# dke-lab/dgll

Hardware: AMD Instinct MI355X
Metric: aggregated edges/sec + epoch time, 3-layer GraphSAGE ogbn-products, 1/2/4/8 GPU (higher is better)
Workload: dtype bf16

## Files before the change

dgll_amd/csrc/gather.hpp:

```cpp
#pragma once
#include "common.hpp"

int dgll_spmm_csr_impl(void* stream, const dgll_csr_plan* plan, const int64_t* rowptr, const int32_t* col,
                       const float* val, const void* X, int64_t ldx, int x_dtype, void* Y, int64_t ldy,
                       int y_dtype, int64_t n_rows, int64_t n_cols, int feat, int reduce, int epilogue,
                       const float* bias, void* workspace, size_t workspace_bytes, const float* row_scale, int accumulate,
                       const void* gate, int64_t ldg, int only_long);

namespace dgll {

template <typename XT, int EPV, int LPR, bool HAS_VAL, int U>
__device__ __forceinline__ void gather_edges(const int32_t* __restrict__ col, const float* __restrict__ val,
                                             const XT* __restrict__ xcol, int64_t ldx, int64_t b, int64_t e,
                                             int lane, float (&acc)[EPV], bool preloaded = false, int first_col = 0,
                                             float first_val = 0.0f) {
    typedef VecIO<XT, EPV> IO;
    constexpr int SLOTS = kWave / LPR;
    const int slot = lane / LPR;

    int my_col = first_col;
    float my_val = first_val;
    if (!preloaded) {
        my_col = 0;
        my_val = 0.0f;
        if (b + lane < e) {
            my_col = __builtin_nontemporal_load(col + b + lane);
            if (HAS_VAL) my_val = __builtin_nontemporal_load(val + b + lane);
        }
    }
    for (int64_t k0 = b; k0 < e; k0 += kWave) {
        const int64_t left = e - k0;
        const int nb = left < kWave ? (int)left : kWave;
        const int cur_col = my_col;
        const float cur_val = my_val;
        const int64_t kn = k0 + kWave + lane;
        if (kn < e) {
            my_col = __builtin_nontemporal_load(col + kn);
            if (HAS_VAL) my_val = __builtin_nontemporal_load(val + kn);
        }
        const uint32_t ld32 = (uint32_t)ldx;
        int j = 0;
        for (; j + SLOTS * U <= nb; j += SLOTS * U) {
            int c[U];
            float w[U];
#pragma unroll
            for (int u = 0; u < U; ++u) {
                const int src = j + u * SLOTS + slot;
                c[u] = __shfl(cur_col, src);
                w[u] = HAS_VAL ? __shfl(cur_val, src) : 1.0f;
            }
            typename IO::raw_t v[U];
#pragma unroll
            for (int u = 0; u < U; ++u) v[u] = IO::load(xcol + (uint64_t)(uint32_t)c[u] * ld32);
#pragma unroll
            for (int u = 0; u < U; ++u) {
                float f[EPV];
                IO::unpack(v[u], f);
#pragma unroll
                for (int i = 0; i < EPV; ++i) acc[i] = HAS_VAL ? fmaf(w[u], f[i], acc[i]) : acc[i] + f[i];
            }
        }
        if (j < nb) {
            int c[U];
            float w[U];
            bool ok[U];
#pragma unroll
            for (int u = 0; u < U; ++u) {
                const int idx = j + u * SLOTS + slot;
                ok[u] = idx < nb;
                const int src = ok[u] ? idx : nb - 1;
                c[u] = __shfl(cur_col, src);
                w[u] = HAS_VAL ? __shfl(cur_val, src) : 1.0f;
            }
            typename IO::raw_t v[U];
#pragma unroll
            for (int u = 0; u < U; ++u) v[u] = IO::load(xcol + (uint64_t)(uint32_t)c[u] * ld32);
#pragma unroll
            for (int u = 0; u < U; ++u) {
                float f[EPV];
                IO::unpack(ok[u] ? v[u] : IO::zero(), f);
#pragma unroll
                for (int i = 0; i < EPV; ++i) acc[i] = HAS_VAL ? fmaf(w[u], f[i], acc[i]) : acc[i] + f[i];
            }
        }
    }
#pragma unroll
    for (int off = LPR; off < kWave; off <<= 1) {
#pragma unroll
        for (int i = 0; i < EPV; ++i) acc[i] += __shfl_xor(acc[i], off);
    }
}

}
```

dgll_amd/csrc/spmm.hip:

```cpp
#include <algorithm>
#include <vector>

#include "common.hpp"
#include "gather.hpp"
#include <type_traits>

namespace dgll {

struct LongRow { int64_t row, begin, end; };

__global__ void find_long_rows_kernel(const int64_t* __restrict__ rowptr, int64_t n_rows, int threshold,
                                      LongRow* __restrict__ out, unsigned long long* __restrict__ count,
                                      unsigned long long capacity) {
    for (int64_t r = blockIdx.x * (int64_t)blockDim.x + threadIdx.x; r < n_rows; r += (int64_t)gridDim.x * blockDim.x) {
        const int64_t b = rowptr[r], e = rowptr[r + 1];
        if (e - b > threshold) {
            const unsigned long long at = atomicAdd(count, 1ull);
            if (at < capacity) out[at] = LongRow{r, b, e};
        }
    }
}

constexpr int64_t kFlatRowCost = 4;
__global__ void flat_row0_kernel(const int64_t* __restrict__ rowptr, int64_t n_rows, int64_t cost_per_wave, int64_t n_flat,
// ... 102 lines not shown
        if (vec_bias) v += bv[i];
        else if ((epilogue & DGLL_EPI_BIAS) && c0 + i < feat) v += bias[c0 + i];
        if (epilogue & DGLL_EPI_RELU) v = fmaxf(v, 0.0f);
        acc[i] = v;
    }
    if constexpr (EXTRA) {
        if (gate) {
            float gv[EPV];
            if (full) gatev.unpack(gv);
#pragma unroll
            for (int i = 0; i < EPV; ++i) {
                if (full) { if (!(gv[i] > 0.0f)) acc[i] = 0.0f; }
                else if (c0 + i < feat && !(load_one<YT>(gate + c0 + i) > 0.0f)) acc[i] = 0.0f;
            }
        }
        if (accumulate == 2) {
            float p[EPV];
            if (full) prev.unpack(p);
#pragma unroll
            for (int i = 0; i < EPV; ++i)
                if (full) acc[i] += p[i];
                else if (c0 + i < feat) acc[i] += load_one<YT>(y + c0 + i);
        }
    }
    if (full) {
        if constexpr (std::is_same<YT, bf16_t>::value && EPV == 8) {
            VecIO<YT, EPV>::store_nt(y + c0, acc);
        } else {
            VecIO<YT, EPV>::store(y + c0, acc);
        }
    } else {
#pragma unroll
        for (int i = 0; i < EPV; ++i)
            if (c0 + i < feat) store_one<YT>(y + c0 + i, acc[i]);
    }
}

template <typename XT, typename YT, int EPV, int LPR, bool HAS_VAL, int U, bool EXTRA, bool PF = false>
__global__ __launch_bounds__(kBlock) void spmm_csr_kernel(const SpmmArgs a) {
    const int lane = lane_id();
    const int wave = __builtin_amdgcn_readfirstlane((int)(threadIdx.x >> 6));
    const int sub = lane % LPR;
    const int c0 = ((int)blockIdx.y * LPR + sub) * EPV;
    const bool col_ok = c0 < a.feat;
    const XT* xcol = static_cast<const XT*>(a.X) + (col_ok ? c0 : 0);
    uint32_t bid = blockIdx.x;

    if (bid < a.chunk_blocks) {
        const int64_t chunk = __builtin_amdgcn_readfirstlane((int)(bid * kWavesPerBlock + wave));
        if (chunk >= a.n_chunks) return;
        float acc[EPV];
#pragma unroll
        for (int i = 0; i < EPV; ++i) acc[i] = 0.0f;
        gather_edges<XT, EPV, LPR, HAS_VAL, U>(a.col, a.val, xcol, a.ldx, uniform64(a.chunk_begin[chunk]),
                                               uniform64(a.chunk_end[chunk]), lane, acc);
        if (lane < LPR && col_ok) {
            float* w = a.ws + chunk * a.ws_ld + c0;
#pragma unroll
            for (int i = 0; i < EPV; ++i) w[i] = acc[i];
        }
        return;
    }

    bid -= a.chunk_blocks;
    if (a.flags & 1) bid = xcd_remap(bid, a.row_blocks);
    const int64_t row0 = ((int64_t)bid * kWavesPerBlock + wave) * a.rows_per_wave;
    constexpr bool pf = PF;
    int64_t nb_ = 0, ne_ = 0;
    int ncol = 0;
    float nval = 0.0f;
    if (pf && row0 < a.n_rows) {
        nb_ = uniform64(a.rowptr[row0]); ne_ = uniform64(a.rowptr[row0 + 1]);
        if (nb_ + lane < ne_) {
            ncol = __builtin_nontemporal_load(a.col + nb_ + lane);
            if (HAS_VAL) nval = __builtin_nontemporal_load(a.val + nb_ + lane);
        }
    }
    for (int r = 0; r < a.rows_per_wave; ++r) {
        const int64_t row = row0 + r;
        if (row >= a.n_rows) return;
        int64_t b, e;
        int fcol = 0;
        float fval = 0.0f;
        if (pf) {
            b = nb_; e = ne_; fcol = ncol; fval = nval;
            if (r + 1 < a.rows_per_wave && row + 1 < a.n_rows) {
                nb_ = e; ne_ = uniform64(a.rowptr[row + 2]);
                ncol = 0; nval = 0.0f;
                if (nb_ + lane < ne_) {
                    ncol = __builtin_nontemporal_load(a.col + nb_ + lane);
                    if (HAS_VAL) nval = __builtin_nontemporal_load(a.val + nb_ + lane);
                }
            }
        } else {
            b = uniform64(a.rowptr[row]); e = uniform64(a.rowptr[row + 1]);
        }
        if (a.threshold > 0 && e - b > a.threshold) continue;
        if constexpr (EXTRA) {
            if (a.accumulate == 2 && e == b) continue;
        }
        float acc[EPV];
#pragma unroll
        for (int i = 0; i < EPV; ++i) acc[i] = 0.0f;
        YT* yrow = static_cast<YT*>(a.Y) + row * a.ldy;
        const bool writer = lane < LPR && col_ok;
        const bool full = c0 + EPV <= a.feat;
        RowVec<YT, EPV> prev, gatev;
        const YT* grow = nullptr;
        if constexpr (EXTRA) {
            grow = a.gate ? static_cast<const YT*>(a.gate) + row * a.ldg : nullptr;
        }
        gather_edges<XT, EPV, LPR, HAS_VAL, U>(a.col, a.val, xcol, a.ldx, b, e, lane, acc, pf, fcol, fval);
        if constexpr (EXTRA) {
            if (writer && full) {
                if (a.accumulate) prev.load(yrow + c0);
                if (grow) gatev.load(grow + c0);
            }
        }
        if (writer) {
            const float scale = a.row_scale ? a.row_scale[row]
                                            : ((a.reduce == DGLL_REDUCE_MEAN && e > b) ? 1.0f / (float)(e - b) : 1.0f);
            finish_row<YT, EPV, EXTRA>(yrow, c0, a.feat, scale, a.epilogue, a.bias, acc, a.accumulate, grow, full, prev, gatev);
        }
    }
}

template <typename XT, typename YT, int EPV, int LPR, bool HAS_VAL, int U, bool EXTRA>
__global__ __launch_bounds__(kBlock) void spmm_csr_flat_kernel(const SpmmArgs a) {
    typedef VecIO<XT, EPV> IO;
    constexpr int SLOTS = kWave / LPR, G = SLOTS * U;
    const int lane = lane_id();
    const int wave = __builtin_amdgcn_readfirstlane((int)(threadIdx.x >> 6));
    const int sub = lane % LPR, slot = lane / LPR;
    const int c0 = ((int)blockIdx.y * LPR + sub) * EPV;
    const bool col_ok = c0 < a.feat;
    const XT* xcol = static_cast<const XT*>(a.X) + (col_ok ? c0 : 0);
    uint32_t bid = blockIdx.x;

    if (bid < a.chunk_blocks) {
        const int64_t chunk = __builtin_amdgcn_readfirstlane((int)(bid * kWavesPerBlock + wave));
        if (chunk >= a.n_chunks) return;
        float acc[EPV];
#pragma unroll
        for (int i = 0; i < EPV; ++i) acc[i] = 0.0f;
        gather_edges<XT, EPV, LPR, HAS_VAL, U>(a.col, a.val, xcol, a.ldx, uniform64(a.chunk_begin[chunk]),
                                               uniform64(a.chunk_end[chunk]), lane, acc);
        if (lane < LPR && col_ok) {
            float* w = a.ws + chunk * a.ws_ld + c0;
#pragma unroll
            for (int i = 0; i < EPV; ++i) w[i] = acc[i];
        }
        return;
    }
    bid -= a.chunk_blocks;
    const int64_t w = (int64_t)bid * kWavesPerBlock + wave;
    if (w >= a.n_flat) return;
    int64_t r = uniform64(a.flat_row0[w]);
    const int64_t r_end = uniform64(a.flat_row0[w + 1]);
    if (r >= r_end) return;
    int64_t rb = uniform64(a.rowptr[r]), re = uniform64(a.rowptr[r + 1]);
    const int64_t p_end = uniform64(a.rowptr[r_end]);
    int64_t p = rb;
    const bool writer = lane < LPR && col_ok;
    const bool full = c0 + EPV <= a.feat;
    const uint32_t ld32 = (uint32_t)a.ldx;
    const int thr = a.threshold;
    float acc[EPV];
#pragma unroll
    for (int i = 0; i < EPV; ++i) acc[i] = 0.0f;
    bool stop = false;

    auto flush = [&]() {
#pragma unroll
        for (int off = LPR; off < kWave; off <<= 1) {
#pragma unroll
            for (int i = 0; i < EPV; ++i) acc[i] += __shfl_xor(acc[i], off);
        }
        bool emit = writer;
        if constexpr (EXTRA) {
            if (a.accumulate == 2 && re == rb) emit = false;
        }
        if (emit) {
            YT* yrow = static_cast<YT*>(a.Y) + r * a.ldy;
            RowVec<YT, EPV> prev, gatev;
            const YT* grow = nullptr;
            if constexpr (EXTRA) {
                grow = a.gate ? static_cast<const YT*>(a.gate) + r * a.ldg : nullptr;
                if (full) {
                    if (a.accumulate) prev.load(yrow + c0);
                    if (grow) gatev.load(grow + c0);
                }
            }
            const float scale = a.row_scale ? a.row_scale[r]
                                            : ((a.reduce == DGLL_REDUCE_MEAN && re > rb) ? 1.0f / (float)(re - rb) : 1.0f);
            finish_row<YT, EPV, EXTRA>(yrow, c0, a.feat, scale, a.epilogue, a.bias, acc, a.accumulate, grow, full, prev, gatev);
        }
#pragma unroll
        for (int i = 0; i < EPV; ++i) acc[i] = 0.0f;
        ++r;
        rb = re;
        if (r < r_end) {
            re = uniform64(a.rowptr[r + 1]);
            stop = thr > 0 && re - rb > thr;
        } else {
            stop = true;
        }
    };

    stop = thr > 0 && re - rb > thr;
    int my_col = 0, nx_col = 0;
    float my_val = 0.0f, nx_val = 0.0f;
    int64_t nx_p = -1;
    while (r < r_end) {
        if (stop) {
            p = re;
            ++r;
            rb = re;
            stop = false;
            if (r < r_end) {
                re = uniform64(a.rowptr[r + 1]);
                stop = thr > 0 && re - rb > thr;
            }
            continue;
        }
        if (re == rb) {
            flush();
            continue;
        }
        const int64_t left = p_end - p;
        const int nb = left < kWave ? (int)left : kWave;
        if (nx_p == p) {
            my_col = nx_col;
            my_val = nx_val;
        } else {
            my_col = 0;
            my_val = 0.0f;
            if (lane < nb) {
                my_col = __builtin_nontemporal_load(a.col + p + lane);
                if (HAS_VAL) my_val = __builtin_nontemporal_load(a.val + p + lane);
            }
        }
        nx_p = p + kWave;
        nx_col = 0;
        nx_val = 0.0f;
        if (nx_p + lane < p_end) {
            nx_col = __builtin_nontemporal_load(a.col + nx_p + lane);
            if (HAS_VAL) nx_val = __builtin_nontemporal_load(a.val + nx_p + lane);
        }
        int j = 0;
        while (j < nb && !stop) {
            const int64_t q0 = p + j;
            const int64_t in_row = re - q0;
            int cnt = nb - j < G ? nb - j : G;
            if (in_row < cnt) cnt = (int)in_row;
            if (cnt == G) {
                int c[U];
                float wv[U];
#pragma unroll
                for (int u = 0; u < U; ++u) {
                    const int src = j + u * SLOTS + slot;
                    c[u] = __shfl(my_col, src);
                    wv[u] = HAS_VAL ? __shfl(my_val, src) : 1.0f;
                }
                typename IO::raw_t v[U];
#pragma unroll
                for (int u = 0; u < U; ++u) v[u] = IO::load(xcol + (uint64_t)(uint32_t)c[u] * ld32);
#pragma unroll
                for (int u = 0; u < U; ++u) {
                    float f[EPV];
                    IO::unpack(v[u], f);
#pragma unroll
                    for (int i = 0; i < EPV; ++i) acc[i] = HAS_VAL ? fmaf(wv[u], f[i], acc[i]) : acc[i] + f[i];
                }
            } else {
                int c[U];
                float wv[U];
                bool ok[U];
#pragma unroll
                for (int u = 0; u < U; ++u) {
                    const int idx = u * SLOTS + slot;
                    ok[u] = idx < cnt;
                    const int src = j + (ok[u] ? idx : cnt - 1);
                    c[u] = __shfl(my_col, src);
                    wv[u] = HAS_VAL ? __shfl(my_val, src) : 1.0f;
                }
                typename IO::raw_t v[U];
#pragma unroll
                for (int u = 0; u < U; ++u) v[u] = IO::load(xcol + (uint64_t)(uint32_t)c[u] * ld32);
#pragma unroll
                for (int u = 0; u < U; ++u) {
                    float f[EPV];
                    IO::unpack(ok[u] ? v[u] : IO::zero(), f);
#pragma unroll
                    for (int i = 0; i < EPV; ++i) acc[i] = HAS_VAL ? fmaf(wv[u], f[i], acc[i]) : acc[i] + f[i];
                }
            }
            j += cnt;
            if (q0 + cnt == re) {
                flush();
                while (!stop && re == rb) flush();
            }
        }
        p = stop ? rb : p + j;
    }
}

template <typename XT, typename YT, int EPV, int LPR, bool HAS_VAL, bool EXTRA>
__global__ __launch_bounds__(kBlock) void spmm_rowslot_kernel(const SpmmArgs a) {
    typedef VecIO<XT, EPV> IO;
    constexpr int SLOTS = kWave / LPR;
    constexpr int U = 4;
    const int lane = lane_id();
    const int wave = __builtin_amdgcn_readfirstlane((int)(threadIdx.x >> 6));
    const int sub = lane % LPR, slot = lane / LPR;
    const int c0 = ((int)blockIdx.y * LPR + sub) * EPV;
    const bool col_ok = c0 < a.feat;
    const XT* xcol = static_cast<const XT*>(a.X) + (col_ok ? c0 : 0);
    uint32_t bid = blockIdx.x;

    if (bid < a.chunk_blocks) {
        const int64_t chunk = __builtin_amdgcn_readfirstlane((int)(bid * kWavesPerBlock + wave));
        if (chunk >= a.n_chunks) return;
        float acc[EPV];
#pragma unroll
        for (int i = 0; i < EPV; ++i) acc[i] = 0.0f;
        gather_edges<XT, EPV, LPR, HAS_VAL, U>(a.col, a.val, xcol, a.ldx, uniform64(a.chunk_begin[chunk]),
                                               uniform64(a.chunk_end[chunk]), lane, acc);
        if (lane < LPR && col_ok) {
            float* w = a.ws + chunk * a.ws_ld + c0;
#pragma unroll
            for (int i = 0; i < EPV; ++i) w[i] = acc[i];
        }
        return;
    }
    bid -= a.chunk_blocks;
    const uint32_t ld32 = (uint32_t)a.ldx;
    const int64_t row0 = ((int64_t)bid * kWavesPerBlock + wave) * a.rows_per_wave;
    for (int r = 0; r < a.rows_per_wave; r += SLOTS) {
        if (row0 + r >= a.n_rows) return;
        const int64_t row = row0 + r + slot;
        int64_t b = 0, e = 0;
        if (row < a.n_rows) { b = a.rowptr[row]; e = a.rowptr[row + 1]; }
        const int64_t full_len = e - b;
        bool mine = row < a.n_rows && !(a.threshold > 0 && full_len > a.threshold);
        if constexpr (EXTRA) {
            if (a.accumulate == 2 && full_len == 0) mine = false;
        }
        const int n = mine ? (int)full_len : 0;
        float acc[EPV];
#pragma unroll
        for (int i = 0; i < EPV; ++i) acc[i] = 0.0f;
        int cnext[U];
        float wnext[U];
#pragma unroll
        for (int u = 0; u < U; ++u) {
            cnext[u] = u < n ? __builtin_nontemporal_load(a.col + b + u) : 0;
            wnext[u] = (HAS_VAL && u < n) ? __builtin_nontemporal_load(a.val + b + u) : 0.0f;
        }
        for (int k = 0; __any(k < n); k += U) {
            int c[U];
            float w[U];
#pragma unroll
            for (int u = 0; u < U; ++u) { c[u] = cnext[u]; w[u] = wnext[u]; }
#pragma unroll
            for (int u = 0; u < U; ++u) {
                const int kn = k + U + u;
                cnext[u] = kn < n ? __builtin_nontemporal_load(a.col + b + kn) : 0;
                wnext[u] = (HAS_VAL && kn < n) ? __builtin_nontemporal_load(a.val + b + kn) : 0.0f;
            }
            typename IO::raw_t v[U];
#pragma unroll
            for (int u = 0; u < U; ++u) v[u] = IO::load(xcol + (uint64_t)(uint32_t)c[u] * ld32);
#pragma unroll
            for (int u = 0; u < U; ++u) {
                float f[EPV];
                IO::unpack(k + u < n ? v[u] : IO::zero(), f);
#pragma unroll
                for (int i = 0; i < EPV; ++i) acc[i] = HAS_VAL ? fmaf(w[u], f[i], acc[i]) : acc[i] + f[i];
            }
        }
        if (!mine || !col_ok) continue;
        YT* yrow = static_cast<YT*>(a.Y) + row * a.ldy;
        const bool full = c0 + EPV <= a.feat;
        RowVec<YT, EPV> prev, gatev;
        const YT* grow = nullptr;
        if constexpr (EXTRA) {
            grow = a.gate ? static_cast<const YT*>(a.gate) + row * a.ldg : nullptr;
            if (full) {
                if (a.accumulate) prev.load(yrow + c0);
                if (grow) gatev.load(grow + c0);
            }
        }
        const float scale = a.row_scale ? a.row_scale[row]
                                        : ((a.reduce == DGLL_REDUCE_MEAN && n > 0) ? 1.0f / (float)n : 1.0f);
        finish_row<YT, EPV, EXTRA>(yrow, c0, a.feat, scale, a.epilogue, a.bias, acc, a.accumulate, grow, full, prev, gatev);
    }
}

template <typename YT>
__global__ __launch_bounds__(kBlock) void spmm_long_finalize_kernel(const SpmmArgs a, const int64_t* __restrict__ long_row,
                                                                    const int32_t* __restrict__ long_chunk0, int64_t n_long) {
    const int lane = lane_id();
    const int64_t li = (int64_t)blockIdx.x * kWavesPerBlock + (threadIdx.x >> 6);
    if (li >= n_long) return;
    const int64_t row = long_row[li];
    const int cb = long_chunk0[li], ce = long_chunk0[li + 1];
    float scale = 1.0f;
    if (a.row_scale) scale = a.row_scale[row];
    else if (a.reduce == DGLL_REDUCE_MEAN) scale = 1.0f / (float)(a.rowptr[row + 1] - a.rowptr[row]);
    YT* y = static_cast<YT*>(a.Y) + row * a.ldy;
    const YT* gate = a.gate ? static_cast<const YT*>(a.gate) + row * a.ldg : nullptr;
    for (int f = lane * 4; f < a.feat; f += kWave * 4) {
        float4 s = make_float4(0.f, 0.f, 0.f, 0.f);
        for (int c = cb; c < ce; c += 8) {
            float4 p[8];
#pragma unroll
            for (int u = 0; u < 8; ++u) {
                const int cc = c + u < ce ? c + u : ce - 1;
                p[u] = *reinterpret_cast<const float4*>(a.ws + (int64_t)cc * a.ws_ld + f);
            }
#pragma unroll
            for (int u = 0; u < 8; ++u)
                if (c + u < ce) { s.x += p[u].x; s.y += p[u].y; s.z += p[u].z; s.w += p[u].w; }
        }
        float v[4] = {s.x, s.y, s.z, s.w};
#pragma unroll
        for (int i = 0; i < 4; ++i) {
            if (f + i >= a.feat) continue;
            float t = v[i];
            if (a.accumulate == 1) t += load_one<YT>(y + f + i);
            t *= scale;
            if (a.epilogue & DGLL_EPI_BIAS) t += a.bias[f + i];
            if (a.epilogue & DGLL_EPI_RELU) t = fmaxf(t, 0.0f);
            if (gate && !(load_one<YT>(gate + f + i) > 0.0f)) t = 0.0f;
            if (a.accumulate == 2) t += load_one<YT>(y + f + i);
            v[i] = t;
        }
        if (f + 4 <= a.feat && (a.flags & 2)) VecIO<YT, 4>::store(y + f, v);
        else
            for (int i = 0; i < 4; ++i) if (f + i < a.feat) store_one<YT>(y + f + i, v[i]);
    }
}

static int ws_ld_for(int feat) { return (feat + 7) & ~7; }

static int g_tune_unroll = 4;
static int g_tune_rows_per_wave = 0;
static int g_tune_flags = 0;
static int g_tune_threshold = 0;
static int g_tune_rowslot = 0;
static int g_tune_flat = 0;
static int g_tune_flat_edges = 256;

template <typename XT, typename YT, int EPV, int LPR, int U>
static hipError_t launch_u(const SpmmArgs& a, dim3 grid, hipStream_t s) {
    const bool extra = a.accumulate || a.gate;
    if constexpr (LPR == 32 && U == 4 && sizeof(XT) == 2 && sizeof(YT) == 2) {
        if (a.flags & 4) {
            if (a.val) {
                if (extra) hipLaunchKernelGGL((spmm_csr_kernel<XT, YT, EPV, LPR, true, U, true, true>), grid, dim3(kBlock), 0, s, a);
                else hipLaunchKernelGGL((spmm_csr_kernel<XT, YT, EPV, LPR, true, U, false, true>), grid, dim3(kBlock), 0, s, a);
            } else {
                if (extra) hipLaunchKernelGGL((spmm_csr_kernel<XT, YT, EPV, LPR, false, U, true, true>), grid, dim3(kBlock), 0, s, a);
                else hipLaunchKernelGGL((spmm_csr_kernel<XT, YT, EPV, LPR, false, U, false, true>), grid, dim3(kBlock), 0, s, a);
            }
            return hipGetLastError();
        }
    }
    if (a.val) {
        if (extra) hipLaunchKernelGGL((spmm_csr_kernel<XT, YT, EPV, LPR, true, U, true>), grid, dim3(kBlock), 0, s, a);
        else hipLaunchKernelGGL((spmm_csr_kernel<XT, YT, EPV, LPR, true, U, false>), grid, dim3(kBlock), 0, s, a);
    } else {
        if (extra) hipLaunchKernelGGL((spmm_csr_kernel<XT, YT, EPV, LPR, false, U, true>), grid, dim3(kBlock), 0, s, a);
        else hipLaunchKernelGGL((spmm_csr_kernel<XT, YT, EPV, LPR, false, U, false>), grid, dim3(kBlock), 0, s, a);
    }
    return hipGetLastError();
}

template <typename XT, typename YT, int EPV, int LPR>
static hipError_t launch_variant(const SpmmArgs& a, dim3 grid, hipStream_t s) {
    if constexpr (LPR >= 32 && EPV > 1) {
        if (g_tune_unroll == 8) return launch_u<XT, YT, EPV, LPR, 8>(a, grid, s);
        if (g_tune_unroll == 2) return launch_u<XT, YT, EPV, LPR, 2>(a, grid, s);
    }
    return launch_u<XT, YT, EPV, LPR, 4>(a, grid, s);
}

template <typename XT, typename YT, int EPV, int LPR>
static hipError_t launch_rowslot(const SpmmArgs& a, dim3 grid, hipStream_t s) {
    const bool extra = a.accumulate || a.gate;
    if (a.val) {
        if (extra) hipLaunchKernelGGL((spmm_rowslot_kernel<XT, YT, EPV, LPR, true, true>), grid, dim3(kBlock), 0, s, a);
        else hipLaunchKernelGGL((spmm_rowslot_kernel<XT, YT, EPV, LPR, true, false>), grid, dim3(kBlock), 0, s, a);
    } else {
        if (extra) hipLaunchKernelGGL((spmm_rowslot_kernel<XT, YT, EPV, LPR, false, true>), grid, dim3(kBlock), 0, s, a);
        else hipLaunchKernelGGL((spmm_rowslot_kernel<XT, YT, EPV, LPR, false, false>), grid, dim3(kBlock), 0, s, a);
    }
    return hipGetLastError();
}

template <typename XT, typename YT, int EPV>
static hipError_t launch_rowslot_lpr(const SpmmArgs& a, int lpr, dim3 grid, hipStream_t s) {
    switch (lpr) {
        case 4: return launch_rowslot<XT, YT, EPV, 4>(a, grid, s);
        case 8: return launch_rowslot<XT, YT, EPV, 8>(a, grid, s);
        case 16: return launch_rowslot<XT, YT, EPV, 16>(a, grid, s);
        default: return launch_rowslot<XT, YT, EPV, 32>(a, grid, s);
    }
}

template <typename XT, typename YT, int EPV, int LPR>
static hipError_t launch_flat(const SpmmArgs& a, dim3 grid, hipStream_t s) {
    const bool extra = a.accumulate || a.gate;
    if (a.val) {
        if (extra) hipLaunchKernelGGL((spmm_csr_flat_kernel<XT, YT, EPV, LPR, true, 4, true>), grid, dim3(kBlock), 0, s, a);
        else hipLaunchKernelGGL((spmm_csr_flat_kernel<XT, YT, EPV, LPR, true, 4, false>), grid, dim3(kBlock), 0, s, a);
    } else {
        if (extra) hipLaunchKernelGGL((spmm_csr_flat_kernel<XT, YT, EPV, LPR, false, 4, true>), grid, dim3(kBlock), 0, s, a);
        else hipLaunchKernelGGL((spmm_csr_flat_kernel<XT, YT, EPV, LPR, false, 4, false>), grid, dim3(kBlock), 0, s, a);
    }
    return hipGetLastError();
}

template <typename XT, typename YT, int EPV>
static hipError_t launch_flat_lpr(const SpmmArgs& a, int lpr, dim3 grid, hipStream_t s) {
    if (lpr == 16) return launch_flat<XT, YT, EPV, 16>(a, grid, s);
    return launch_flat<XT, YT, EPV, 32>(a, grid, s);
}

template <typename XT, typename YT, int EPV>
static hipError_t launch_lpr(const SpmmArgs& a, int lpr, dim3 grid, hipStream_t s) {
    switch (lpr) {
        case 4: return launch_variant<XT, YT, EPV, 4>(a, grid, s);
        case 8: return launch_variant<XT, YT, EPV, 8>(a, grid, s);
        case 16: return launch_variant<XT, YT, EPV, 16>(a, grid, s);
        case 32: return launch_variant<XT, YT, EPV, 32>(a, grid, s);
        default: return launch_variant<XT, YT, EPV, 64>(a, grid, s);
    }
}

}

using namespace dgll;

DGLL_API int dgll_hip_csr_plan_create(void* stream, const int64_t* rowptr, int64_t n_rows, int64_t nnz,
                                      int long_row_threshold, dgll_csr_plan** out_plan) {
    DGLL_REQUIRE(out_plan != nullptr, "out_plan is NULL");
    DGLL_REQUIRE(rowptr != nullptr && n_rows >= 0 && nnz >= 0, "bad CSR arguments");
    hipStream_t s = static_cast<hipStream_t>(stream);
    dgll_csr_plan* p = new dgll_csr_plan();
    p->n_rows = n_rows;
    p->nnz = nnz;
    p->threshold = long_row_threshold > 0 ? long_row_threshold : (g_tune_threshold > 0 ? g_tune_threshold : 256);
    hipError_t e = hipGetDevice(&p->device);
    if (e != hipSuccess) { delete p; return hip_fail(e, "hipGetDevice"); }
    if (long_row_threshold < 0) {
        p->threshold = 0;
        *out_plan = p;
        return DGLL_OK;
    }

// ... 40 lines not shown
        for (int64_t b = h_list[i].begin; b < h_list[i].end; b += p->threshold) {
            chunk_begin.push_back(b);
            chunk_end.push_back(std::min<int64_t>(b + p->threshold, h_list[i].end));
            chunk_row.push_back(h_list[i].row);
        }
    }
    chunk0[h_count] = (int32_t)chunk_begin.size();
    p->n_long = (int64_t)h_count;
    p->n_chunks = (int64_t)chunk_begin.size();
    if (p->n_long > 0) {
        PLAN_TRY(hipMalloc(&p->d_long_row, sizeof(int64_t) * h_count));
        PLAN_TRY(hipMalloc(&p->d_long_chunk0, sizeof(int32_t) * (h_count + 1)));
        PLAN_TRY(hipMalloc(&p->d_chunk_begin, sizeof(int64_t) * chunk_begin.size()));
        PLAN_TRY(hipMalloc(&p->d_chunk_end, sizeof(int64_t) * chunk_end.size()));
        PLAN_TRY(hipMalloc(&p->d_chunk_row, sizeof(int64_t) * chunk_row.size()));
        PLAN_TRY(hipMemcpyAsync(p->d_chunk_row, chunk_row.data(), sizeof(int64_t) * chunk_row.size(), hipMemcpyHostToDevice, s));
        PLAN_TRY(hipMemcpyAsync(p->d_long_row, long_row.data(), sizeof(int64_t) * h_count, hipMemcpyHostToDevice, s));
        PLAN_TRY(hipMemcpyAsync(p->d_long_chunk0, chunk0.data(), sizeof(int32_t) * (h_count + 1), hipMemcpyHostToDevice, s));
        PLAN_TRY(hipMemcpyAsync(p->d_chunk_begin, chunk_begin.data(), sizeof(int64_t) * chunk_begin.size(), hipMemcpyHostToDevice, s));
        PLAN_TRY(hipMemcpyAsync(p->d_chunk_end, chunk_end.data(), sizeof(int64_t) * chunk_end.size(), hipMemcpyHostToDevice, s));
        PLAN_TRY(hipStreamSynchronize(s));
    }
    if (n_rows > 0 && g_tune_flat_edges > 0) {
        p->flat_edges = g_tune_flat_edges;
        p->n_flat = (nnz + kFlatRowCost * n_rows + p->flat_edges - 1) / p->flat_edges;
        PLAN_TRY(hipMalloc(&p->d_flat_row0, sizeof(int64_t) * (size_t)(p->n_flat + 1)));
        const int blocks = (int)std::min<int64_t>((p->n_flat + 1 + kBlock - 1) / kBlock, 4096);
        hipLaunchKernelGGL(flat_row0_kernel, dim3(blocks), dim3(kBlock), 0, s, rowptr, n_rows, (int64_t)p->flat_edges, p->n_flat,
                           p->d_flat_row0);
        PLAN_TRY(hipGetLastError());
        PLAN_TRY(hipStreamSynchronize(s));
    }
#undef PLAN_TRY
    cleanup();
    *out_plan = p;
    return DGLL_OK;
}

extern int g_tune_mfma_kperm;
extern int g_tune_gat_gen;
extern int g_tune_res_per_cu;
extern int g_tune_loader_blocks_per_cu;

DGLL_API int dgll_hip_debug_tune(int key, int value) {
    switch (key) {
        case 0: g_tune_unroll = value; break;
        case 1: g_tune_rows_per_wave = value; break;
        case 2: g_tune_flags = value; break;
        case 3: g_tune_threshold = value; break;
        case 4: g_tune_mfma_kperm = value; break;
        case 5: g_tune_rowslot = value; break;
        case 13: g_tune_flat = value; break;
        case 14: g_tune_flat_edges = value; break;
        case 7: break;
        case 9: g_tune_gat_gen = value; break;
        case 11: g_tune_res_per_cu = value; break;
        case 12: g_tune_loader_blocks_per_cu = value; break;
        default: set_error("unknown tuning key"); return DGLL_ERR_INVALID;
    }
    return DGLL_OK;
}

DGLL_API void dgll_hip_csr_plan_destroy(dgll_csr_plan* p) {
    if (!p) return;
    if (p->d_long_row) (void)hipFree(p->d_long_row);
    if (p->d_long_chunk0) (void)hipFree(p->d_long_chunk0);
    if (p->d_chunk_begin) (void)hipFree(p->d_chunk_begin);
    if (p->d_chunk_end) (void)hipFree(p->d_chunk_end);
    if (p->d_chunk_row) (void)hipFree(p->d_chunk_row);
    if (p->d_flat_row0) (void)hipFree(p->d_flat_row0);
    delete p;
}

DGLL_API size_t dgll_hip_csr_plan_workspace_bytes(const dgll_csr_plan* p, int feat) {
    if (!p || p->n_chunks == 0 || feat <= 0) return 0;
    return (size_t)p->n_chunks * (size_t)ws_ld_for(feat) * sizeof(float);
}

DGLL_API int64_t dgll_hip_csr_plan_num_long_rows(const dgll_csr_plan* p) { return p ? p->n_long : 0; }
DGLL_API int64_t dgll_hip_csr_plan_num_chunks(const dgll_csr_plan* p) { return p ? p->n_chunks : 0; }


DGLL_API int dgll_hip_spmm_csr(void* stream, const dgll_csr_plan* plan, const int64_t* rowptr, const int32_t* col,
                               const float* val, const void* X, int64_t ldx, int x_dtype, void* Y, int64_t ldy,
                               int y_dtype, int64_t n_rows, int64_t n_cols, int feat, int reduce, int epilogue,
                               const float* bias, void* workspace, size_t workspace_bytes) {
    return dgll_spmm_csr_impl(stream, plan, rowptr, col, val, X, ldx, x_dtype, Y, ldy, y_dtype, n_rows, n_cols, feat, reduce,
                              epilogue, bias, workspace, workspace_bytes, nullptr, 0, nullptr, 0, 0);
}

DGLL_API int dgll_hip_spmm_csr_ex(void* stream, const dgll_csr_plan* plan, const int64_t* rowptr, const int32_t* col,
                                  const float* val, const void* X, int64_t ldx, int x_dtype, void* Y, int64_t ldy,
                                  int y_dtype, int64_t n_rows, int64_t n_cols, int feat, int reduce, int epilogue,
                                  const float* bias, void* workspace, size_t workspace_bytes, const float* row_scale,
                                  int accumulate) {
    return dgll_spmm_csr_impl(stream, plan, rowptr, col, val, X, ldx, x_dtype, Y, ldy, y_dtype, n_rows, n_cols, feat, reduce,
                              epilogue, bias, workspace, workspace_bytes, row_scale, accumulate, nullptr, 0, 0);
}

DGLL_API int dgll_hip_spmm_csr_gated(void* stream, const dgll_csr_plan* plan, const int64_t* rowptr, const int32_t* col,
                                     const float* val, const void* X, int64_t ldx, int x_dtype, void* Y, int64_t ldy,
                                     int y_dtype, int64_t n_rows, int64_t n_cols, int feat, int reduce, int epilogue,
                                     const float* bias, void* workspace, size_t workspace_bytes, const float* row_scale,
                                     int accumulate, const void* gate, int64_t ldg) {
    return dgll_spmm_csr_impl(stream, plan, rowptr, col, val, X, ldx, x_dtype, Y, ldy, y_dtype, n_rows, n_cols, feat, reduce,
                              epilogue, bias, workspace, workspace_bytes, row_scale, accumulate, gate, ldg, 0);
// ... 33 lines not shown
    a.accumulate = accumulate;
    a.gate = gate; a.ldg = ldg;
    if (plan) {
        DGLL_REQUIRE(plan->n_rows == n_rows, "plan was built for a different CSR");
        a.threshold = plan->threshold;
        a.n_chunks = plan->n_chunks;
        a.chunk_begin = plan->d_chunk_begin;
        a.chunk_end = plan->d_chunk_end;
        if (plan->n_chunks > 0) {
            const size_t need = dgll_hip_csr_plan_workspace_bytes(plan, feat);
            if (!workspace || workspace_bytes < need) {
                set_error("workspace too small for the plan's long-row partials");
                return DGLL_ERR_WORKSPACE;
            }
            a.ws = static_cast<float*>(workspace);
        }
        const double row_bytes = (double)plan->nnz / (double)std::max<int64_t>(n_rows, 1) * feat *
                                 (x_dtype == DGLL_BF16 ? 2.0 : 4.0);
        int rpw = row_bytes > 0 ? (int)(98304.0 / row_bytes) : 8;
        a.rows_per_wave = std::min(std::max(rpw, 1), 8);
        if (g_tune_rows_per_wave > 0) a.rows_per_wave = g_tune_rows_per_wave;
    }
    if (only_long && (!plan || plan->n_long == 0)) return DGLL_OK;
    const int64_t waves = (n_rows + a.rows_per_wave - 1) / a.rows_per_wave;
    const int64_t row_blocks = only_long ? 0 : (waves + kWavesPerBlock - 1) / kWavesPerBlock;
    int64_t chunk_blocks = (a.n_chunks + kWavesPerBlock - 1) / kWavesPerBlock;
    chunk_blocks = (chunk_blocks + kXcds - 1) / kXcds * kXcds;
    DGLL_REQUIRE(row_blocks + chunk_blocks < (int64_t)0x7fffffff, "grid too large");
    a.row_blocks = (uint32_t)row_blocks;
    a.chunk_blocks = (uint32_t)chunk_blocks;

    const int esz = x_dtype == DGLL_BF16 ? 2 : 4;
    const int ysz = y_dtype == DGLL_BF16 ? 2 : 4;
    const int epv = 16 / esz;
    const bool fast = aligned16(X) && aligned16(Y) && (ldx * esz) % 16 == 0 && (ldy * ysz) % 16 == 0 &&
                      ((int64_t)epv * ysz) % 16 == 0 && (!gate || (aligned16(gate) && (ldg * ysz) % 16 == 0));
    if (fast) a.flags |= 2;
    hipError_t err;
    bool rowslot = false;
    if (fast) {
        const int vecs = (feat + epv - 1) / epv;
        int lpr = 4;
        while (lpr < 64 && lpr < vecs) lpr <<= 1;
        const double avg_len = plan ? (double)plan->nnz / (double)std::max<int64_t>(n_rows, 1) : 1e9;
        rowslot = !only_long && lpr <= 32 && g_tune_rowslot != 1 &&
                  (g_tune_rowslot == 2 || (lpr <= 16 && avg_len <= 24.0) || (lpr == 32 && avg_len <= 4.5));
        if (rowslot) {
            const int slots = kWave / lpr;
            a.rows_per_wave = std::max(a.rows_per_wave, 1);
            a.rows_per_wave = (a.rows_per_wave + slots - 1) / slots * slots;
            if (g_tune_rows_per_wave > 0) a.rows_per_wave = (g_tune_rows_per_wave + slots - 1) / slots * slots;
        }
    }
    if (rowslot) {
        const int64_t waves2 = (n_rows + a.rows_per_wave - 1) / a.rows_per_wave;
        const int64_t row_blocks2 = (waves2 + kWavesPerBlock - 1) / kWavesPerBlock;
        DGLL_REQUIRE(row_blocks2 + chunk_blocks < (int64_t)0x7fffffff, "grid too large");
        a.row_blocks = (uint32_t)row_blocks2;
        const int vecs = (feat + epv - 1) / epv;
        int lpr = 4;
        while (lpr < 64 && lpr < vecs) lpr <<= 1;
        dim3 grid((uint32_t)(row_blocks2 + chunk_blocks), (uint32_t)((vecs + lpr - 1) / lpr));
        if (x_dtype == DGLL_F32) err = launch_rowslot_lpr<float, float, 4>(a, lpr, grid, s);
        else if (y_dtype == DGLL_BF16) err = launch_rowslot_lpr<bf16_t, bf16_t, 8>(a, lpr, grid, s);
        else err = launch_rowslot_lpr<bf16_t, float, 8>(a, lpr, grid, s);
    } else if (fast && !only_long && plan && plan->d_flat_row0 && g_tune_flat != 1 && g_tune_unroll == 4 && !(a.flags & 1) &&
               [&]() { const int v = (feat + epv - 1) / epv; return v > 8 && v <= 32; }() &&
               (g_tune_flat == 2 || (x_dtype == DGLL_F32 && (double)plan->nnz / (double)std::max<int64_t>(n_rows, 1) >= 8.0))) {
        const int vecs = (feat + epv - 1) / epv;
        const int lpr = vecs <= 16 ? 16 : 32;
        a.flat_row0 = plan->d_flat_row0;
        a.n_flat = plan->n_flat;
        const int64_t flat_blocks = (plan->n_flat + kWavesPerBlock - 1) / kWavesPerBlock;
        DGLL_REQUIRE(flat_blocks + chunk_blocks < (int64_t)0x7fffffff, "grid too large");
        a.row_blocks = (uint32_t)flat_blocks;
        dim3 grid((uint32_t)(flat_blocks + chunk_blocks), (uint32_t)((vecs + lpr - 1) / lpr));
        if (x_dtype == DGLL_F32) err = launch_flat_lpr<float, float, 4>(a, lpr, grid, s);
        else if (y_dtype == DGLL_BF16) err = launch_flat_lpr<bf16_t, bf16_t, 8>(a, lpr, grid, s);
        else err = launch_flat_lpr<bf16_t, float, 8>(a, lpr, grid, s);
    } else if (fast) {
        const int vecs = (feat + epv - 1) / epv;
        int lpr = 4;
        while (lpr < 64 && lpr < vecs) lpr <<= 1;
        dim3 grid((uint32_t)(row_blocks + chunk_blocks), (uint32_t)((vecs + lpr - 1) / lpr));
        if (x_dtype == DGLL_F32) err = launch_lpr<float, float, 4>(a, lpr, grid, s);
        else if (y_dtype == DGLL_BF16) err = launch_lpr<bf16_t, bf16_t, 8>(a, lpr, grid, s);
        else err = launch_lpr<bf16_t, float, 8>(a, lpr, grid, s);
    } else {
        dim3 grid((uint32_t)(row_blocks + chunk_blocks), (uint32_t)((feat + 63) / 64));
        if (x_dtype == DGLL_F32) err = launch_variant<float, float, 1, 64>(a, grid, s);
        else if (y_dtype == DGLL_BF16) err = launch_variant<bf16_t, bf16_t, 1, 64>(a, grid, s);
        else err = launch_variant<bf16_t, float, 1, 64>(a, grid, s);
    }
    if (err != hipSuccess) return hip_fail(err, "spmm_csr_kernel launch");

    if (plan && plan->n_long > 0) {
        dim3 grid((uint32_t)((plan->n_long + kWavesPerBlock - 1) / kWavesPerBlock));
        if (y_dtype == DGLL_F32)
            hipLaunchKernelGGL(spmm_long_finalize_kernel<float>, grid, dim3(kBlock), 0, s, a, plan->d_long_row,
                               plan->d_long_chunk0, plan->n_long);
        else
            hipLaunchKernelGGL(spmm_long_finalize_kernel<bf16_t>, grid, dim3(kBlock), 0, s, a, plan->d_long_row,
                               plan->d_long_chunk0, plan->n_long);
        err = hipGetLastError();
        if (err != hipSuccess) return hip_fail(err, "spmm_long_finalize_kernel launch");
    }
    return DGLL_OK;
// ... 2 lines not shown
```

Measured before the change: 30.97 billion.

## Use DPP/permlane slot reduction and scalar constant loads in SpMM kernels

```diff
diff --git a/dgll_amd/csrc/gather.hpp b/dgll_amd/csrc/gather.hpp
--- a/dgll_amd/csrc/gather.hpp
+++ b/dgll_amd/csrc/gather.hpp
@@ -8,6 +8,38 @@
                        const void* gate, int64_t ldg, int only_long);
 
 namespace dgll {
+
+__device__ __forceinline__ int64_t load_uniform(const int64_t* p, int64_t i) {
+    return ((const __attribute__((address_space(4))) int64_t*)p)[i];
+}
+
+template <int OFF>
+__device__ __forceinline__ float row_ror(float v) {
+    return __builtin_bit_cast(float, __builtin_amdgcn_update_dpp(0, __builtin_bit_cast(int, v), 0x120 + OFF, 0xf, 0xf, false));
+}
+
+__device__ __forceinline__ float from_odd_row(float v) {
+    const unsigned u = __builtin_bit_cast(unsigned, v);
+    return __builtin_bit_cast(float, (unsigned)__builtin_amdgcn_permlane16_swap(u, u, false, false)[1]);
+}
+
+__device__ __forceinline__ float from_upper_half(float v) {
+    const unsigned u = __builtin_bit_cast(unsigned, v);
+    return __builtin_bit_cast(float, (unsigned)__builtin_amdgcn_permlane32_swap(u, u, false, false)[1]);
+}
+
+template <int EPV, int LPR>
+__device__ __forceinline__ void reduce_slots(float (&acc)[EPV]) {
+#pragma unroll
+    for (int i = 0; i < EPV; ++i) {
+        if constexpr (LPR <= 1) acc[i] += row_ror<1>(acc[i]);
+        if constexpr (LPR <= 2) acc[i] += row_ror<2>(acc[i]);
+        if constexpr (LPR <= 4) acc[i] += row_ror<4>(acc[i]);
+        if constexpr (LPR <= 8) acc[i] += row_ror<8>(acc[i]);
+        if constexpr (LPR <= 16) acc[i] += from_odd_row(acc[i]);
+        if constexpr (LPR <= 32) acc[i] += from_upper_half(acc[i]);
+    }
+}
 
 template <typename XT, int EPV, int LPR, bool HAS_VAL, int U>
 __device__ __forceinline__ void gather_edges(const int32_t* __restrict__ col, const float* __restrict__ val,
@@ -84,11 +116,7 @@
             }
         }
     }
-#pragma unroll
-    for (int off = LPR; off < kWave; off <<= 1) {
-#pragma unroll
-        for (int i = 0; i < EPV; ++i) acc[i] += __shfl_xor(acc[i], off);
-    }
+    reduce_slots<EPV, LPR>(acc);
 }
 
 }
diff --git a/dgll_amd/csrc/spmm.hip b/dgll_amd/csrc/spmm.hip
--- a/dgll_amd/csrc/spmm.hip
+++ b/dgll_amd/csrc/spmm.hip
@@ -178,8 +178,8 @@
         float acc[EPV];
 #pragma unroll
         for (int i = 0; i < EPV; ++i) acc[i] = 0.0f;
-        gather_edges<XT, EPV, LPR, HAS_VAL, U>(a.col, a.val, xcol, a.ldx, uniform64(a.chunk_begin[chunk]),
-                                               uniform64(a.chunk_end[chunk]), lane, acc);
+        gather_edges<XT, EPV, LPR, HAS_VAL, U>(a.col, a.val, xcol, a.ldx, load_uniform(a.chunk_begin, chunk),
+                                               load_uniform(a.chunk_end, chunk), lane, acc);
         if (lane < LPR && col_ok) {
             float* w = a.ws + chunk * a.ws_ld + c0;
 #pragma unroll
@@ -191,40 +191,39 @@
     bid -= a.chunk_blocks;
     if (a.flags & 1) bid = xcd_remap(bid, a.row_blocks);
     const int64_t row0 = ((int64_t)bid * kWavesPerBlock + wave) * a.rows_per_wave;
+    if (row0 >= a.n_rows) return;
+    const int64_t row_end = row0 + a.rows_per_wave < a.n_rows ? row0 + a.rows_per_wave : a.n_rows;
     constexpr bool pf = PF;
-    int64_t nb_ = 0, ne_ = 0;
     int ncol = 0;
     float nval = 0.0f;
-    if (pf && row0 < a.n_rows) {
-        nb_ = uniform64(a.rowptr[row0]); ne_ = uniform64(a.rowptr[row0 + 1]);
-        if (nb_ + lane < ne_) {
-            ncol = __builtin_nontemporal_load(a.col + nb_ + lane);
-            if (HAS_VAL) nval = __builtin_nontemporal_load(a.val + nb_ + lane);
-        }
-    }
-    for (int r = 0; r < a.rows_per_wave; ++r) {
+    bool pre = false;
+    auto request = [&](int64_t qb, int64_t qe) {
+        ncol = 0;
+        nval = 0.0f;
+        if (qb + lane < qe) {
+            ncol = __builtin_nontemporal_load(a.col + qb + lane);
+            if (HAS_VAL) nval = __builtin_nontemporal_load(a.val + qb + lane);
+        }
+        pre = true;
+    };
+    const int nr = (int)(row_end - row0);
+    int64_t nb = load_uniform(a.rowptr, row0), ne = load_uniform(a.rowptr, row0 + 1);
+    if (pf) request(nb, ne);
+    for (int r = 0; r < nr; ++r) {
         const int64_t row = row0 + r;
-        if (row >= a.n_rows) return;
-        int64_t b, e;
-        int fcol = 0;
-        float fval = 0.0f;
-        if (pf) {
-            b = nb_; e = ne_; fcol = ncol; fval = nval;
-            if (r + 1 < a.rows_per_wave && row + 1 < a.n_rows) {
-                nb_ = e; ne_ = uniform64(a.rowptr[row + 2]);
-                ncol = 0; nval = 0.0f;
-                if (nb_ + lane < ne_) {
-                    ncol = __builtin_nontemporal_load(a.col + nb_ + lane);
-                    if (HAS_VAL) nval = __builtin_nontemporal_load(a.val + nb_ + lane);
-                }
-            }
-        } else {
-            b = uniform64(a.rowptr[row]); e = uniform64(a.rowptr[row + 1]);
-        }
+        const int64_t b = nb, e = ne;
+        const bool has_next = r + 1 < nr;
+        nb = e;
+        if (has_next) ne = load_uniform(a.rowptr, row + 2);
+        const bool cur_pre = pre;
+        const int fcol = ncol;
+        const float fval = nval;
+        pre = false;
         if (a.threshold > 0 && e - b > a.threshold) continue;
         if constexpr (EXTRA) {
             if (a.accumulate == 2 && e == b) continue;
         }
+        if (pf && has_next) request(nb, ne);
         float acc[EPV];
 #pragma unroll
         for (int i = 0; i < EPV; ++i) acc[i] = 0.0f;
@@ -236,7 +235,7 @@
         if constexpr (EXTRA) {
             grow = a.gate ? static_cast<const YT*>(a.gate) + row * a.ldg : nullptr;
         }
-        gather_edges<XT, EPV, LPR, HAS_VAL, U>(a.col, a.val, xcol, a.ldx, b, e, lane, acc, pf, fcol, fval);
+        gather_edges<XT, EPV, LPR, HAS_VAL, U>(a.col, a.val, xcol, a.ldx, b, e, lane, acc, cur_pre, fcol, fval);
         if constexpr (EXTRA) {
             if (writer && full) {
                 if (a.accumulate) prev.load(yrow + c0);
@@ -269,8 +268,8 @@
         float acc[EPV];
 #pragma unroll
         for (int i = 0; i < EPV; ++i) acc[i] = 0.0f;
-        gather_edges<XT, EPV, LPR, HAS_VAL, U>(a.col, a.val, xcol, a.ldx, uniform64(a.chunk_begin[chunk]),
-                                               uniform64(a.chunk_end[chunk]), lane, acc);
+        gather_edges<XT, EPV, LPR, HAS_VAL, U>(a.col, a.val, xcol, a.ldx, load_uniform(a.chunk_begin, chunk),
+                                               load_uniform(a.chunk_end, chunk), lane, acc);
         if (lane < LPR && col_ok) {
             float* w = a.ws + chunk * a.ws_ld + c0;
 #pragma unroll
@@ -281,11 +280,11 @@
     bid -= a.chunk_blocks;
     const int64_t w = (int64_t)bid * kWavesPerBlock + wave;
     if (w >= a.n_flat) return;
-    int64_t r = uniform64(a.flat_row0[w]);
-    const int64_t r_end = uniform64(a.flat_row0[w + 1]);
+    int64_t r = load_uniform(a.flat_row0, w);
+    const int64_t r_end = load_uniform(a.flat_row0, w + 1);
     if (r >= r_end) return;
-    int64_t rb = uniform64(a.rowptr[r]), re = uniform64(a.rowptr[r + 1]);
-    const int64_t p_end = uniform64(a.rowptr[r_end]);
+    int64_t rb = load_uniform(a.rowptr, r), re = load_uniform(a.rowptr, r + 1);
+    const int64_t p_end = load_uniform(a.rowptr, r_end);
     int64_t p = rb;
     const bool writer = lane < LPR && col_ok;
     const bool full = c0 + EPV <= a.feat;
@@ -297,11 +296,7 @@
     bool stop = false;
 
     auto flush = [&]() {
-#pragma unroll
-        for (int off = LPR; off < kWave; off <<= 1) {
-#pragma unroll
-            for (int i = 0; i < EPV; ++i) acc[i] += __shfl_xor(acc[i], off);
-        }
+        reduce_slots<EPV, LPR>(acc);
         bool emit = writer;
         if constexpr (EXTRA) {
             if (a.accumulate == 2 && re == rb) emit = false;
@@ -326,7 +321,7 @@
         ++r;
         rb = re;
         if (r < r_end) {
-            re = uniform64(a.rowptr[r + 1]);
+            re = load_uniform(a.rowptr, r + 1);
             stop = thr > 0 && re - rb > thr;
         } else {
             stop = true;
@@ -344,7 +339,7 @@
             rb = re;
             stop = false;
             if (r < r_end) {
-                re = uniform64(a.rowptr[r + 1]);
+                re = load_uniform(a.rowptr, r + 1);
                 stop = thr > 0 && re - rb > thr;
             }
             continue;
@@ -450,8 +445,8 @@
         float acc[EPV];
 #pragma unroll
         for (int i = 0; i < EPV; ++i) acc[i] = 0.0f;
-        gather_edges<XT, EPV, LPR, HAS_VAL, U>(a.col, a.val, xcol, a.ldx, uniform64(a.chunk_begin[chunk]),
-                                               uniform64(a.chunk_end[chunk]), lane, acc);
+        gather_edges<XT, EPV, LPR, HAS_VAL, U>(a.col, a.val, xcol, a.ldx, load_uniform(a.chunk_begin, chunk),
+                                               load_uniform(a.chunk_end, chunk), lane, acc);
         if (lane < LPR && col_ok) {
             float* w = a.ws + chunk * a.ws_ld + c0;
 #pragma unroll
```

New measurement: 31.18 billion (median of 6 runs). No clear change (+0.7%).

## Add row-group SpMM kernel splitting each row across multiple wave slots

Applied to the files above, without the earlier changes.

```diff
diff --git a/dgll_amd/csrc/gather.hpp b/dgll_amd/csrc/gather.hpp
--- a/dgll_amd/csrc/gather.hpp
+++ b/dgll_amd/csrc/gather.hpp
@@ -91,4 +91,111 @@
     }
 }
 
-}
+template <int OFF> __device__ __forceinline__ float xor_lane(float v) {
+    if constexpr (OFF == 8) return __int_as_float(__builtin_amdgcn_update_dpp(0, __float_as_int(v), 0x128 , 0xf, 0xf, false));
+    else return __shfl_xor(v, OFF);
+}
+
+template <typename XT, int EPV>
+__device__ __forceinline__ void unpack_if(const typename VecIO<XT, EPV>::raw_t& r, bool ok, float (&f)[EPV]) {
+    if constexpr (sizeof(XT) == 2 && EPV == 8) {
+        const uint32_t lo = ok ? 0x01000c0cu : 0x0c0c0c0cu, hi = ok ? 0x03020c0cu : 0x0c0c0c0cu;
+        const uint32_t d[4] = {r.x, r.y, r.z, r.w};
+#pragma unroll
+        for (int i = 0; i < 4; ++i) {
+            f[2 * i] = __uint_as_float(__builtin_amdgcn_perm(0u, d[i], lo));
+            f[2 * i + 1] = __uint_as_float(__builtin_amdgcn_perm(0u, d[i], hi));
+        }
+    } else {
+        VecIO<XT, EPV>::unpack(ok ? r : VecIO<XT, EPV>::zero(), f);
+    }
+}
+
+template <typename XT, int EPV, int LPR, int SPR, bool HAS_VAL, int U>
+__device__ __forceinline__ void gather_edges_grouped(const int32_t* __restrict__ col, const float* __restrict__ val,
+                                                     const XT* __restrict__ xcol, uint32_t ld32, int64_t b, int n, int lane,
+                                                     float (&acc)[EPV]) {
+    typedef VecIO<XT, EPV> IO;
+    constexpr int SLOTS = kWave / LPR, G = SLOTS / SPR, GL = SPR * LPR, UL = U / G, R = SPR * U;
+    static_assert(SLOTS % SPR == 0 && G >= 1 && U % G == 0 && GL % R == 0, "row-group geometry");
+    const int gl = lane % GL, gbase = lane - gl, q = gl / LPR;
+    const int64_t off = b + gl;
+
+    int nmax = 0;
+#pragma unroll
+    for (int g = 0; g < G; ++g) nmax = max(nmax, __builtin_amdgcn_readlane(n, g * GL));
+
+    int my_col = 0;
+    float my_val = 0.0f;
+    if (gl < n) {
+        my_col = __builtin_nontemporal_load(col + off);
+        if (HAS_VAL) my_val = __builtin_nontemporal_load(val + off);
+    }
+    for (int kb = 0; kb < nmax; kb += GL) {
+        const int cur_col = my_col;
+        const float cur_val = my_val;
+        if (kb + GL + gl < n) {
+            my_col = __builtin_nontemporal_load(col + off + kb + GL);
+            if (HAS_VAL) my_val = __builtin_nontemporal_load(val + off + kb + GL);
+        }
+#pragma unroll 1
+        for (int j = 0; j < GL && kb + j < nmax; j += R) {
+            int c[U];
+            float w[U];
+            bool ok[U];
+#pragma unroll
+            for (int m = 0; m < U; ++m) {
+                const int idx = j + (m % UL) * SLOTS + q * G + m / UL;
+                ok[m] = kb + idx < n;
+                c[m] = __shfl(cur_col, gbase + idx);
+                w[m] = HAS_VAL ? __shfl(cur_val, gbase + idx) : 1.0f;
+            }
+            typename IO::raw_t v[U];
+#pragma unroll
+            for (int m = 0; m < U; ++m) v[m] = IO::load(xcol + (uint64_t)(uint32_t)c[m] * ld32);
+            float t[G][EPV];
+#pragma unroll
+            for (int g = 0; g < G; ++g) {
+#pragma unroll
+                for (int l = 0; l < UL; ++l) {
+                    const int m = g * UL + l;
+                    float f[EPV];
+                    unpack_if<XT, EPV>(v[m], ok[m], f);
+#pragma unroll
+                    for (int i = 0; i < EPV; ++i) {
+                        if (l == 0) t[g][i] = HAS_VAL ? fmaf(w[m], f[i], 0.0f) : f[i];
+                        else t[g][i] = HAS_VAL ? fmaf(w[m], f[i], t[g][i]) : t[g][i] + f[i];
+                    }
+                }
+                if constexpr (G >= 2) {
+                    if (g % 2 == 1) {
+#pragma unroll
+                        for (int i = 0; i < EPV; ++i) t[g - 1][i] += t[g][i];
+                        __builtin_amdgcn_sched_barrier(0);
+                    }
+                }
+            }
+#pragma unroll
+            for (int s = 2; s < G; s <<= 1) {
+#pragma unroll
+                for (int g = 0; g < G; g += 2 * s) {
+#pragma unroll
+                    for (int i = 0; i < EPV; ++i) t[g][i] += t[g + s][i];
+                }
+            }
+#pragma unroll
+            for (int i = 0; i < EPV; ++i) acc[i] += t[0][i];
+        }
+    }
+    if constexpr (SPR >= 2) {
+#pragma unroll
+        for (int i = 0; i < EPV; ++i) acc[i] += xor_lane<LPR>(acc[i]);
+    }
+    if constexpr (SPR >= 4) {
+#pragma unroll
+        for (int i = 0; i < EPV; ++i) acc[i] += xor_lane<2 * LPR>(acc[i]);
+    }
+    static_assert(SPR <= 4, "row-group kernel: 2 or 4 slots per row");
+}
+
+}
diff --git a/dgll_amd/csrc/spmm.hip b/dgll_amd/csrc/spmm.hip
--- a/dgll_amd/csrc/spmm.hip
+++ b/dgll_amd/csrc/spmm.hip
@@ -523,6 +523,58 @@
     }
 }
 
+template <typename XT, typename YT, int EPV, int LPR, int SPR, bool HAS_VAL>
+__global__ __launch_bounds__(kBlock) void spmm_rowgroup_kernel(const SpmmArgs a) {
+    constexpr int SLOTS = kWave / LPR, G = SLOTS / SPR, GL = kWave / G, U = 4;
+    const int lane = lane_id();
+    const int wave = __builtin_amdgcn_readfirstlane((int)(threadIdx.x >> 6));
+    const int sub = lane % LPR, grp = lane / GL;
+    const int c0 = ((int)blockIdx.y * LPR + sub) * EPV;
+    const bool col_ok = c0 < a.feat;
+    const XT* xcol = static_cast<const XT*>(a.X) + (col_ok ? c0 : 0);
+    uint32_t bid = blockIdx.x;
+
+    if (bid < a.chunk_blocks) {
+        const int64_t chunk = __builtin_amdgcn_readfirstlane((int)(bid * kWavesPerBlock + wave));
+        if (chunk >= a.n_chunks) return;
+        float acc[EPV];
+#pragma unroll
+        for (int i = 0; i < EPV; ++i) acc[i] = 0.0f;
+        gather_edges<XT, EPV, LPR, HAS_VAL, U>(a.col, a.val, xcol, a.ldx, uniform64(a.chunk_begin[chunk]),
+                                               uniform64(a.chunk_end[chunk]), lane, acc);
+        if (lane < LPR && col_ok) {
+            float* w = a.ws + chunk * a.ws_ld + c0;
+#pragma unroll
+            for (int i = 0; i < EPV; ++i) w[i] = acc[i];
+        }
+        return;
+    }
+    bid -= a.chunk_blocks;
+    const uint32_t ld32 = (uint32_t)a.ldx;
+    const bool writer = col_ok && lane % GL < LPR;
+    const bool full = c0 + EPV <= a.feat;
+    const int64_t row0 = ((int64_t)bid * kWavesPerBlock + wave) * a.rows_per_wave;
+    for (int r = 0; r < a.rows_per_wave; r += G) {
+        if (row0 + r >= a.n_rows) return;
+        const int64_t row = row0 + r + grp;
+        int64_t b = 0, e = 0;
+        if (row < a.n_rows) { b = a.rowptr[row]; e = a.rowptr[row + 1]; }
+        const int64_t full_len = e - b;
+        const bool mine = row < a.n_rows && !(a.threshold > 0 && full_len > a.threshold);
+        const int n = mine ? (int)full_len : 0;
+        float acc[EPV];
+#pragma unroll
+        for (int i = 0; i < EPV; ++i) acc[i] = 0.0f;
+        gather_edges_grouped<XT, EPV, LPR, SPR, HAS_VAL, U>(a.col, a.val, xcol, ld32, b, n, lane, acc);
+        if (!mine || !writer) continue;
+        YT* yrow = static_cast<YT*>(a.Y) + row * a.ldy;
+        RowVec<YT, EPV> prev, gatev;
+        const float scale = a.row_scale ? a.row_scale[row]
+                                        : ((a.reduce == DGLL_REDUCE_MEAN && n > 0) ? 1.0f / (float)n : 1.0f);
+        finish_row<YT, EPV, false>(yrow, c0, a.feat, scale, a.epilogue, a.bias, acc, 0, nullptr, full, prev, gatev);
+    }
+}
+
 template <typename YT>
 __global__ __launch_bounds__(kBlock) void spmm_long_finalize_kernel(const SpmmArgs a, const int64_t* __restrict__ long_row,
                                                                     const int32_t* __restrict__ long_chunk0, int64_t n_long) {
@@ -569,6 +621,7 @@
 }
 
 static int ws_ld_for(int feat) { return (feat + 7) & ~7; }
+constexpr double kRowGroupMaxAvgLen8 = 100.0, kRowGroupMaxAvgLen16 = 64.0;
 
 static int g_tune_unroll = 4;
 static int g_tune_rows_per_wave = 0;
@@ -577,6 +630,7 @@
 static int g_tune_rowslot = 0;
 static int g_tune_flat = 0;
 static int g_tune_flat_edges = 256;
+static int g_tune_rowgroup = 0;
 
 template <typename XT, typename YT, int EPV, int LPR, int U>
 static hipError_t launch_u(const SpmmArgs& a, dim3 grid, hipStream_t s) {
@@ -633,6 +687,20 @@
         case 16: return launch_rowslot<XT, YT, EPV, 16>(a, grid, s);
         default: return launch_rowslot<XT, YT, EPV, 32>(a, grid, s);
     }
+}
+
+template <typename XT, typename YT, int EPV, int LPR, int SPR>
+static hipError_t launch_rowgroup(const SpmmArgs& a, dim3 grid, hipStream_t s) {
+    if (a.val) hipLaunchKernelGGL((spmm_rowgroup_kernel<XT, YT, EPV, LPR, SPR, true>), grid, dim3(kBlock), 0, s, a);
+    else hipLaunchKernelGGL((spmm_rowgroup_kernel<XT, YT, EPV, LPR, SPR, false>), grid, dim3(kBlock), 0, s, a);
+    return hipGetLastError();
+}
+
+template <typename YT>
+static hipError_t launch_rowgroup_lpr(const SpmmArgs& a, int lpr, int spr, dim3 grid, hipStream_t s) {
+    if (lpr == 16) return launch_rowgroup<bf16_t, YT, 8, 16, 2>(a, grid, s);
+    if (spr == 4) return launch_rowgroup<bf16_t, YT, 8, 8, 4>(a, grid, s);
+    return launch_rowgroup<bf16_t, YT, 8, 8, 2>(a, grid, s);
 }
 
 template <typename XT, typename YT, int EPV, int LPR>
@@ -779,6 +847,7 @@
         case 5: g_tune_rowslot = value; break;
         case 13: g_tune_flat = value; break;
         case 14: g_tune_flat_edges = value; break;
+        case 15: g_tune_rowgroup = value; break;
         case 7: break;
         case 9: g_tune_gat_gen = value; break;
         case 11: g_tune_res_per_cu = value; break;
@@ -918,7 +987,32 @@
             if (g_tune_rows_per_wave > 0) a.rows_per_wave = (g_tune_rows_per_wave + slots - 1) / slots * slots;
         }
     }
-    if (rowslot) {
+    int rowgroup_spr = 0;
+    if (fast && !rowslot && !only_long && x_dtype == DGLL_BF16 && !accumulate && !gate && g_tune_rowgroup != 1 &&
+        g_tune_unroll == 4 && !(a.flags & 1)) {
+        const int vecs = (feat + epv - 1) / epv;
+        const double avg_len = plan ? (double)plan->nnz / (double)std::max<int64_t>(n_rows, 1) : 1e9;
+        if (g_tune_rowgroup == 2 || g_tune_rowgroup == 4) {
+            if (vecs > 4 && vecs <= 8) rowgroup_spr = g_tune_rowgroup;
+            else if (vecs > 8 && vecs <= 16) rowgroup_spr = 2;
+        } else if (avg_len > 24.0 && ((vecs > 4 && vecs <= 8 && avg_len <= kRowGroupMaxAvgLen8) ||
+                                      (vecs > 8 && vecs <= 16 && avg_len <= kRowGroupMaxAvgLen16))) {
+            rowgroup_spr = 2;
+        }
+    }
+    if (rowgroup_spr) {
+        const int vecs = (feat + epv - 1) / epv;
+        const int lpr = vecs <= 8 ? 8 : 16;
+        const int rows = kWave / lpr / rowgroup_spr;
+        a.rows_per_wave = (std::max(a.rows_per_wave, 1) + rows - 1) / rows * rows;
+        const int64_t waves2 = (n_rows + a.rows_per_wave - 1) / a.rows_per_wave;
+        const int64_t row_blocks2 = (waves2 + kWavesPerBlock - 1) / kWavesPerBlock;
+        DGLL_REQUIRE(row_blocks2 + chunk_blocks < (int64_t)0x7fffffff, "grid too large");
+        a.row_blocks = (uint32_t)row_blocks2;
+        dim3 grid((uint32_t)(row_blocks2 + chunk_blocks), 1u);
+        if (y_dtype == DGLL_BF16) err = launch_rowgroup_lpr<bf16_t>(a, lpr, rowgroup_spr, grid, s);
+        else err = launch_rowgroup_lpr<float>(a, lpr, rowgroup_spr, grid, s);
+    } else if (rowslot) {
         const int64_t waves2 = (n_rows + a.rows_per_wave - 1) / a.rows_per_wave;
         const int64_t row_blocks2 = (waves2 + kWavesPerBlock - 1) / kWavesPerBlock;
         DGLL_REQUIRE(row_blocks2 + chunk_blocks < (int64_t)0x7fffffff, "grid too large");
```

After: 30.89 billion before, 32.72 billion after (median of 6 runs). 5.9% higher.
